# Shuijing725/CrowdNav_Prediction_AttnGraph

Measured on AMD Instinct MI355X. Metric: env-steps/sec (sim+policy fwd) at 20 humans, higher is better.
Workload: dtype f32 (big GEMMs as bf16x3 split-precision MFMA, fp32 accumulate); 1 GPU; BASELINE configs[1]: CrowdSimVarNum-v0, 20 humans, 4096 parallel envs per GPU, HH+HR attention on, policy forward + ORCA sim step + auto-reset per step; envs_per_gpu=4096, humans=20, parallelism=dp1 (envs sharded, no rollout collective), policy_init=orthogonal, torch.manual_seed(425), sampled_actions=True, side_stream_tail=inline, dephase_steps=240

## Files before the change

crowdnav_prediction_attngraph_amd/csrc/orca.h:

```cpp
#pragma once
#include "env_dev.h"
#include "det_math.h"

namespace {

struct LpLine { float px, py, dx, dy; };

__device__ __forceinline__ bool wv_any(bool p) { return __ballot(p) != 0ull; }

__device__ __forceinline__ bool lp1_wave(const LpLine &L, uint64_t valid, int i, float ipx, float ipy, float idx, float idy,
                                         float radius, float optx, float opty, bool dirOpt, int lane, float &rx, float &ry)
{
    const float dotProduct = ipx * idx + ipy * idy;
    const float discriminant = dotProduct * dotProduct + radius * radius - (ipx * ipx + ipy * ipy);
    if (discriminant < 0.0f) return false;
    const float sq = sqrtf(discriminant);
    float tLeft = -dotProduct - sq;
    float tRight = -dotProduct + sq;
    const bool mine = lane < i && ((valid >> lane) & 1ull);
    const float denominator = idx * L.dy - idy * L.dx;
    const float numerator = L.dx * (ipy - L.py) - L.dy * (ipx - L.px);
    const bool parallel = fabsf(denominator) <= RVO_EPS;
    const bool pfail = mine && parallel && numerator < 0.0f;
    const float t = numerator / denominator;
    const float candR = (mine && !parallel && denominator >= 0.0f) ? t : INFINITY;
    const float candL = (mine && !parallel && denominator < 0.0f) ? t : -INFINITY;
    tRight = fminf(tRight, wv_min(candR));
    tLeft = fmaxf(tLeft, wv_max(candL));
    if (wv_any(pfail) || tLeft > tRight) return false;
    float t_opt;
    if (dirOpt) {
        t_opt = (optx * idx + opty * idy > 0.0f) ? tRight : tLeft;
    } else {
        const float tt = idx * (optx - ipx) + idy * (opty - ipy);
        t_opt = tt < tLeft ? tLeft : (tt > tRight ? tRight : tt);
    }
    rx = ipx + t_opt * idx;
    ry = ipy + t_opt * idy;
    return true;
}

__device__ __forceinline__ int lp2_wave(const LpLine &L, uint64_t valid, int n, float radius, float optx, float opty,
                                        bool dirOpt, int lane, float &rx, float &ry)
{
    if (dirOpt) {
        rx = radius * optx; ry = radius * opty;
    } else if (optx * optx + opty * opty > radius * radius) {
        const float inv = 1.0f / sqrtf(optx * optx + opty * opty);
        rx = radius * (optx * inv); ry = radius * (opty * inv);
    } else {
        rx = optx; ry = opty;
    }
    uint64_t todo = valid & (n >= 64 ? ~0ull : ((1ull << n) - 1ull));
    for (;;) {
        const uint64_t vm = __ballot(L.dx * (L.py - ry) - L.dy * (L.px - rx) > 0.0f) & todo;
        if (!vm) return n;
        const int i = __builtin_amdgcn_readfirstlane(__ffsll((unsigned long long)vm) - 1);
        todo &= ~((2ull << i) - 1ull);
        const float ipx = wv_readlane(L.px, i), ipy = wv_readlane(L.py, i);
        const float idx = wv_readlane(L.dx, i), idy = wv_readlane(L.dy, i);
        const float tx = rx, ty = ry;
        if (!lp1_wave(L, valid, i, ipx, ipy, idx, idy, radius, optx, opty, dirOpt, lane, rx, ry)) {
            rx = tx; ry = ty;
            return i;
        }
    }
}

__device__ __forceinline__ void lp3_wave(const LpLine &L, int n, int beginLine, float radius, int lane, float &rx, float &ry)
{
    float distance = 0.0f;
    uint64_t todo = (n >= 64 ? ~0ull : ((1ull << n) - 1ull)) & ~((1ull << beginLine) - 1ull);
    for (;;) {
        const uint64_t vm = __ballot(L.dx * (L.py - ry) - L.dy * (L.px - rx) > distance) & todo;
        if (!vm) return;
        const int i = __builtin_amdgcn_readfirstlane(__ffsll((unsigned long long)vm) - 1);
        todo &= ~((2ull << i) - 1ull);
        const float ipx = wv_readlane(L.px, i), ipy = wv_readlane(L.py, i);
        const float idx = wv_readlane(L.dx, i), idy = wv_readlane(L.dy, i);
        LpLine Pj;
        const float determinant = idx * L.dy - idy * L.dx;
        const bool par = fabsf(determinant) <= RVO_EPS;
        const bool skip = par && (idx * L.dx + idy * L.dy > 0.0f);
        if (par) {
            Pj.px = 0.5f * (ipx + L.px); Pj.py = 0.5f * (ipy + L.py);
        } else {
            const float s = (L.dx * (ipy - L.py) - L.dy * (ipx - L.px)) / determinant;
            Pj.px = ipx + s * idx; Pj.py = ipy + s * idy;
        }
        const float ddx = L.dx - idx, ddy = L.dy - idy;
        const float inv = 1.0f / sqrtf(ddx * ddx + ddy * ddy);
        Pj.dx = ddx * inv; Pj.dy = ddy * inv;
        const uint64_t pvalid = __ballot(lane < i && !skip);
        const float tx = rx, ty = ry;
        if (lp2_wave(Pj, pvalid, i, radius, -idy, idx, true, lane, rx, ry) < i) { rx = tx; ry = ty; }
        distance = idx * (ipy - ry) - idy * (ipx - rx);
    }
}

__device__ __forceinline__ uint32_t hw_ballot(bool p, int lane)
{
    const uint64_t b = __ballot(p);
    return (lane & 32) ? (uint32_t)(b >> 32) : (uint32_t)b;
}
__device__ __forceinline__ float hw_read(float v, int lane, int i)
{
    return __int_as_float(__builtin_amdgcn_ds_bpermute(((lane & 32) + i) << 2, __float_as_int(v)));
}
__device__ __forceinline__ float hw_last(float v, int lane)
{
    const float a = wv_readlane(v, 31), b = wv_readlane(v, 63);
    return (lane & 32) ? b : a;
}
__device__ __forceinline__ uint32_t hw_key(float f)
{
    const uint32_t u = __float_as_uint(f);
    return u ^ ((uint32_t)((int32_t)u >> 31) | 0x80000000u);
}
__device__ __forceinline__ float hw_unkey(uint32_t k) { return __uint_as_float(k ^ ((uint32_t)((int32_t)~k >> 31) | 0x80000000u)); }
template <int CTRL, int ROW_MASK>
__device__ __forceinline__ uint32_t hw_dpp(uint32_t v, uint32_t identity)
{
    return (uint32_t)__builtin_amdgcn_update_dpp((int)identity, (int)v, CTRL, ROW_MASK, 0xf, false);
}
__device__ __forceinline__ uint32_t hw_min(uint32_t v, int lane)
{
    v = min(v, hw_dpp<0x111, 0xf>(v, ~0u));
    v = min(v, hw_dpp<0x112, 0xf>(v, ~0u));
    v = min(v, hw_dpp<0x114, 0xf>(v, ~0u));
    v = min(v, hw_dpp<0x118, 0xf>(v, ~0u));
    v = min(v, hw_dpp<0x142, 0xa>(v, ~0u));
    return __float_as_uint(hw_last(__uint_as_float(v), lane));
}
__device__ __forceinline__ uint32_t hw_max(uint32_t v, int lane)
{
    v = max(v, hw_dpp<0x111, 0xf>(v, 0u));
    v = max(v, hw_dpp<0x112, 0xf>(v, 0u));
    v = max(v, hw_dpp<0x114, 0xf>(v, 0u));
    v = max(v, hw_dpp<0x118, 0xf>(v, 0u));
    v = max(v, hw_dpp<0x142, 0xa>(v, 0u));
    return __float_as_uint(hw_last(__uint_as_float(v), lane));
}

struct LpChord { uint32_t kLeft, kRight, inDisc, pickRight; };

__device__ __forceinline__ LpChord lp_chords(const LpLine &L, float radius, float optx, float opty, int lane)
{
    LpChord c;
    const float dotProduct = L.px * L.dx + L.py * L.dy;
    const float discriminant = dotProduct * dotProduct + radius * radius - (L.px * L.px + L.py * L.py);
    const float sq = sqrtf(discriminant);
    c.kLeft = hw_key(-dotProduct - sq);
    c.kRight = hw_key(-dotProduct + sq);
    c.inDisc = hw_ballot(!(discriminant < 0.0f), lane);
    c.pickRight = hw_ballot(optx * L.dx + opty * L.dy > 0.0f, lane);
    return c;
}

__device__ __forceinline__ bool lp1_pair(const LpLine &L, const LpChord &C, uint32_t valid, int i, float ipx, float ipy, float idx, float idy,
                                         bool act, int lane, float &rx, float &ry)
{
    const int hl = lane & 31;
    bool ok = (C.inDisc >> i) & 1u;
    const uint32_t kLeft = __float_as_uint(hw_read(__uint_as_float(C.kLeft), lane, i));
    const uint32_t kRight = __float_as_uint(hw_read(__uint_as_float(C.kRight), lane, i));
    const bool mine = hl < i && ((valid >> hl) & 1u);
    const float denominator = idx * L.dy - idy * L.dx;
    const float numerator = L.dx * (ipy - L.py) - L.dy * (ipx - L.px);
    const bool parallel = fabsf(denominator) <= RVO_EPS;
    const bool pfail = mine && parallel && numerator < 0.0f;
    const float t = numerator / denominator;
    const uint32_t kt = hw_key(t);
    const uint32_t candR = (mine && !parallel && denominator >= 0.0f) ? kt : 0xff800000u;
    const uint32_t candL = (mine && !parallel && denominator < 0.0f) ? kt : 0x007fffffu;
    const float tRight = hw_unkey(min(kRight, hw_min(candR, lane)));
    const float tLeft = hw_unkey(max(kLeft, hw_max(candL, lane)));
    const uint32_t pf = hw_ballot(pfail, lane);
    ok = ok & (pf == 0u) & !(tLeft > tRight);
    const float t_opt = ((C.pickRight >> i) & 1u) ? tRight : tLeft;
    if (act && ok) {
        rx = ipx + t_opt * idx;
        ry = ipy + t_opt * idy;
    }
    return ok;
}

__device__ __forceinline__ int lp2_pair(const LpLine &L, uint32_t valid, int n, float radius, float optx, float opty, bool act, int lane,
                                        float &rx, float &ry)
{
    if (act) { rx = radius * optx; ry = radius * opty; }
    const LpChord C = lp_chords(L, radius, optx, opty, lane);
    uint32_t todo = valid & ((1u << n) - 1u);
    int res = n;
    bool running = act;
    for (;;) {
        const uint32_t vm = hw_ballot(L.dx * (L.py - ry) - L.dy * (L.px - rx) > 0.0f, lane) & todo;
        const bool go = running && vm != 0u;
        if (__ballot(go) == 0ull) return res;
        running = go;
        const int i = go ? __ffs((int)vm) - 1 : 0;
        if (go) todo &= ~((2u << i) - 1u);
        const float ipx = hw_read(L.px, lane, i), ipy = hw_read(L.py, lane, i);
        const float idx = hw_read(L.dx, lane, i), idy = hw_read(L.dy, lane, i);
        const bool ok = lp1_pair(L, C, valid, i, ipx, ipy, idx, idy, go, lane, rx, ry);
        if (go && !ok) { res = i; running = false; }
    }
}

__device__ __forceinline__ void lp3_pair(const LpLine &L, int n, int beginLine, float radius, bool act, int lane, float &rx, float &ry)
{
    const int hl = lane & 31;
    float distance = 0.0f;
    uint32_t todo = (n >= 32 ? ~0u : ((1u << n) - 1u)) & ~((1u << beginLine) - 1u);
    bool running = act;
    for (;;) {
        const uint32_t vm = hw_ballot(L.dx * (L.py - ry) - L.dy * (L.px - rx) > distance, lane) & todo;
        const bool go = running && vm != 0u;
        if (__ballot(go) == 0ull) return;
        running = go;
        const int i = go ? __ffs((int)vm) - 1 : 0;
        if (go) todo &= ~((2u << i) - 1u);
        const float ipx = hw_read(L.px, lane, i), ipy = hw_read(L.py, lane, i);
        const float idx = hw_read(L.dx, lane, i), idy = hw_read(L.dy, lane, i);
        LpLine Pj;
        const float determinant = idx * L.dy - idy * L.dx;
        const bool par = fabsf(determinant) <= RVO_EPS;
        const bool skip = par && (idx * L.dx + idy * L.dy > 0.0f);
        if (par) {
            Pj.px = 0.5f * (ipx + L.px); Pj.py = 0.5f * (ipy + L.py);
        } else {
            const float s = (L.dx * (ipy - L.py) - L.dy * (ipx - L.px)) / determinant;
            Pj.px = ipx + s * idx; Pj.py = ipy + s * idy;
        }
        const float ddx = L.dx - idx, ddy = L.dy - idy;
        const float inv = 1.0f / sqrtf(ddx * ddx + ddy * ddy);
        Pj.dx = ddx * inv; Pj.dy = ddy * inv;
        const uint32_t pvalid = hw_ballot(hl < i && !skip, lane);
        const float tx = rx, ty = ry;
        const int f = lp2_pair(Pj, pvalid, i, radius, -idy, idx, go, lane, rx, ry);
        if (go && f < i) { rx = tx; ry = ty; }
        if (go) distance = idx * (ipy - ry) - idy * (ipx - rx);
    }
}

__global__ __launch_bounds__(256) void orca_lp3_kernel(EnvDev s)
{
    const CnStampScope stamp_scope(s.stamp);
    const int lane = threadIdx.x & 63, hl = lane & 31, half = lane >> 5;
    const int total = *s.lp3_cnt;
    const int pairs = (total + 1) >> 1;
    const int H = s.H;
    for (int p = __builtin_amdgcn_readfirstlane(blockIdx.x * 4 + (threadIdx.x >> 6)); p < pairs; p += gridDim.x * 4) {
        const bool act = 2 * p + half < total;
        const int k = act ? 2 * p + half : 2 * p;
        const Lp3Hdr hd = s.lp3_hdr[k];
        float4 raw = s.lp3_lines[(size_t)k * 32 + hl];
        raw.x = held(raw.x); raw.y = held(raw.y); raw.z = held(raw.z); raw.w = held(raw.w);
        const float4 ln = hl < hd.nn ? raw : make_float4(0.0f, 0.0f, 1.0f, 0.0f);
        LpLine L;
        L.px = ln.x; L.py = ln.y; L.dx = ln.z; L.dy = ln.w;
        float rx = hd.rx, ry = hd.ry;
        lp3_pair(L, hd.nn, hd.line_fail, hd.radius, act, lane, rx, ry);
        if (act && hl == 0) {
            const int e = hd.agent / H, i = hd.agent - e * H;
            s.hact[(size_t)e * 2 * H + i] = rx;
            s.hact[(size_t)e * 2 * H + H + i] = ry;
        }
    }
}

__device__ __forceinline__ void orca_wave(int lane, int nl, bool cand, float opx, float opy, float ovx, float ovy, float orad,
                                          float spx, float spy, float svx, float svy, float srad, float maxspeed, float prefx,
                                          float prefy, float nd, int max_nb, float th, float dt, float &outx, float &outy)
{
    const float ddx0 = spx - opx, ddy0 = spy - opy;
    const float dq = ddx0 * ddx0 + ddy0 * ddy0;
    const bool inrange = cand && dq < nd * nd;
    const float key = inrange ? dq : INFINITY;
    int rank = 0;
    for (int m = 0; m < nl; ++m) {
        const float km = wv_readlane(key, m);
        rank += (km < key || (km == key && m < lane)) ? 1 : 0;
    }
    if (lane >= nl) rank = lane;
    int nn = __popcll(__ballot(inrange));
    if (nn > max_nb) nn = max_nb;
    const float rpx = opx - spx, rpy = opy - spy;
    const float rvx = svx - ovx, rvy = svy - ovy;
    const float distSq = rpx * rpx + rpy * rpy;
    const float cr = srad + orad;
    const float crSq = cr * cr;
    float ldx, ldy, ux, uy;
    if (distSq > crSq) {
        const float invTH = 1.0f / th;
        const float wx = rvx - invTH * rpx, wy = rvy - invTH * rpy;
        const float wLenSq = wx * wx + wy * wy;
        const float dot1 = wx * rpx + wy * rpy;
        if (dot1 < 0.0f && dot1 * dot1 > crSq * wLenSq) {
            const float wLen = sqrtf(wLenSq);
            const float inv = 1.0f / wLen;
            const float uwx = wx * inv, uwy = wy * inv;
            ldx = uwy; ldy = -uwx;
            const float s = cr * invTH - wLen;
            ux = s * uwx; uy = s * uwy;
        } else {
            const float leg = sqrtf(distSq - crSq);
            const float invD = 1.0f / distSq;
            if (rpx * wy - rpy * wx > 0.0f) {
                ldx = (rpx * leg - rpy * cr) * invD;
                ldy = (rpx * cr + rpy * leg) * invD;
            } else {
                ldx = -((rpx * leg + rpy * cr) * invD);
                ldy = -((-rpx * cr + rpy * leg) * invD);
            }
            const float dot2 = rvx * ldx + rvy * ldy;
            ux = dot2 * ldx - rvx; uy = dot2 * ldy - rvy;
        }
    } else {
        const float invDT = 1.0f / dt;
        const float wx = rvx - invDT * rpx, wy = rvy - invDT * rpy;
        const float wLen = sqrtf(wx * wx + wy * wy);
        const float inv = 1.0f / wLen;
        const float uwx = wx * inv, uwy = wy * inv;
        ldx = uwy; ldy = -uwx;
        const float s = cr * invDT - wLen;
        ux = s * uwx; uy = s * uwy;
    }
    const float lpx = svx + 0.5f * ux, lpy = svy + 0.5f * uy;
    LpLine L;
    L.px = __int_as_float(__builtin_amdgcn_ds_permute(rank << 2, __float_as_int(lpx)));
    L.py = __int_as_float(__builtin_amdgcn_ds_permute(rank << 2, __float_as_int(lpy)));
    L.dx = __int_as_float(__builtin_amdgcn_ds_permute(rank << 2, __float_as_int(ldx)));
    L.dy = __int_as_float(__builtin_amdgcn_ds_permute(rank << 2, __float_as_int(ldy)));
    const uint64_t valid = nn >= 64 ? ~0ull : ((1ull << nn) - 1ull);
    float rx, ry;
    const int lineFail = lp2_wave(L, valid, nn, maxspeed, prefx, prefy, false, lane, rx, ry);
    if (lineFail < nn) lp3_wave(L, nn, lineFail, maxspeed, lane, rx, ry);
    outx = rx; outy = ry;
}

__device__ __forceinline__ void orca_agent(const EnvDev &s, int agent, int lane)
{
    const int H = s.H;
    const int e = agent / H, i = agent - e * H;
    const int n = crowd_size(s, e);
    if (i >= n) return;
    const double *hum = s.hum + (size_t)e * 8 * H;
    const bool isH = lane < n;
    const int lj = isH ? lane : 0;
    const double px = hum[F_PX * H + lj], py = hum[F_PY * H + lj], vx = hum[F_VX * H + lj], vy = hum[F_VY * H + lj];
    const double rad = hum[F_RAD * H + lj];
    const double spx = __shfl(px, i, 64), spy = __shfl(py, i, 64), svx = __shfl(vx, i, 64), svy = __shfl(vy, i, 64);
    const double sgx = hum[F_GX * H + i], sgy = hum[F_GY * H + i], srad = hum[F_RAD * H + i], svpref = hum[F_VPREF * H + i];
    const double safety = s.cfg.orca_safety_space;
    const size_t ei = (size_t)e * H + i;
    float nd, self_r, self_ms, seen_r;
    const bool rv = s.cfg.robot_visible != 0;
    const int n_agents = n + (rv ? 1 : 0);
    const bool isR = rv && lane == n;
    const double *rob = s.rob + (size_t)e * 8;
    const double qx = isR ? rob[R_PX] : px, qy = isR ? rob[R_PY] : py, qvx = isR ? rob[R_VX] : vx, qvy = isR ? rob[R_VY] : vy;
    const bool coincident = s.cfg.human_fov < 2.0 ? !in_fov(s.cfg, s.cfg.human_fov, spx, spy, svx, svy, 0.0, qx, qy) : (qx == spx) && (qy == spy);
    if (!s.sim_valid[ei] || (s.sim_n && s.sim_n[ei] != n_agents)) {
        nd = (float)s.shared_nd[e];
        self_r = (float)(srad + 0.01 + safety);
        self_ms = (float)svpref;
        seen_r = (float)((coincident ? s.cfg.human_radius : rad) + 0.01 + safety);
        if (s.sim_seen && isH) s.sim_seen[ei * H + lane] = seen_r;
        if (lane == 0) {
            s.sim_nd[ei] = nd; s.sim_self_radius[ei] = self_r; s.sim_self_maxspeed[ei] = self_ms; s.sim_valid[ei] = 1;
            if (s.sim_n) s.sim_n[ei] = (uint8_t)n_agents;
        }
    } else {
        nd = s.sim_nd[ei]; self_r = s.sim_self_radius[ei]; self_ms = s.sim_self_maxspeed[ei];
        seen_r = s.sim_seen ? s.sim_seen[ei * H + lj] : (float)(rad + 0.01 + safety);
    }
    if (isR) seen_r = (float)(s.cfg.robot_radius + 0.01 + safety);
    const bool cand = (isH && lane != i) || isR;
    const float opx = coincident ? 7.0f : (float)qx, opy = coincident ? 7.0f : (float)qy;
    const float ovx = coincident ? 0.0f : (float)qvx, ovy = coincident ? 0.0f : (float)qvy;
    double gvx = sgx - spx, gvy = sgy - spy;
    const double speed = sqrt(gvx * gvx + gvy * gvy);
    if (speed > 1.0) { gvx = gvx / speed; gvy = gvy / speed; }
    float ox, oy;
    orca_wave(lane, n_agents, cand, opx, opy, ovx, ovy, seen_r, (float)spx, (float)spy, (float)svx, (float)svy, self_r, self_ms,
              (float)gvx, (float)gvy, nd, n_agents - 1, (float)s.cfg.orca_time_horizon, (float)s.cfg.time_step, ox, oy);
    if (lane == 0) {
        s.hact[(size_t)e * 2 * H + i] = ox;
        s.hact[(size_t)e * 2 * H + H + i] = oy;
    }
}

__global__ __launch_bounds__(256) void orca_kernel(EnvDev s)
{
    const CnStampScope stamp_scope(s.stamp);
    const int lane = threadIdx.x & 63;
    const int total = s.E * s.H;
    for (int agent = __builtin_amdgcn_readfirstlane(blockIdx.x * 4 + (threadIdx.x >> 6)); agent < total; agent += gridDim.x * 4)
        orca_agent(s, agent, lane);
}

#include "orca_sortnet.inc"
#include "row_plan.h"

template <int W> struct LaneVec;
template <> struct LaneVec<8> { typedef float f __attribute__((ext_vector_type(8))); };
template <> struct LaneVec<32> { typedef float f __attribute__((ext_vector_type(32))); };

template <int NB, int VW>
__global__ __launch_bounds__(64) void orca_lane_kernel(EnvDev s, const float *plan_det, int32_t *plan, int plan_groups, unsigned long long *plan_stamp)
{
    const CnStampScope stamp_scope((plan && (int)blockIdx.x < plan_groups) ? plan_stamp : s.stamp);
    constexpr int RAW = (int)sizeof(rowplan::Lds) > NB * 64 * 16 ? (int)sizeof(rowplan::Lds) : NB * 64 * 16;
    __shared__ __attribute__((aligned(16))) char s_raw[RAW];
    if (plan && (int)blockIdx.x < plan_groups) {
        __builtin_amdgcn_s_setprio(3);
        rowplan::build((int)blockIdx.x, plan_groups, s.E, s.H, rp_workgroups(s.E, s.H), plan_det, plan, *reinterpret_cast<rowplan::Lds *>(s_raw), nullptr, s.plan_arrive);
        return;
    }
    const int blk = (int)blockIdx.x - (plan ? plan_groups : 0);
    typedef typename LaneVec<VW>::f vec;
    const int agent = blk * 64 + threadIdx.x;
    const int H = s.H;
    const bool live_lane = agent < s.E * H;
    const int e = live_lane ? agent / H : (blk * 64) / H, i = live_lane ? agent - e * H : 0;
    const int n = crowd_size(s, e);
    const bool active = live_lane && i < n;
    const cn_env_config &c = s.cfg;
    constexpr int NENV = NB == 8 ? 65 : (NB == 20 ? 10 : 5);
    __shared__ double s_px[128], s_py[128], s_vx[128], s_vy[128], s_rad[128], s_rob[NENV][4];
    const double *hum = s.hum + (size_t)e * 8 * H;
    const size_t ei = (size_t)e * H + i;
    double sgx, sgy, svpref, shared_nd_in;
    int sim_valid_in, sim_n_in = 0;
    float sim_nd_in, sim_r_in, sim_ms_in;
    {
        const int a0 = blk * 64;
        const int e0 = a0 / H, e1 = (min(a0 + 63, s.E * H - 1)) / H;
        const int nrows = (e1 - e0 + 1) * H;
        double st[2][5];
#pragma unroll
        for (int it = 0; it < 2; ++it) {
            const int r = threadIdx.x + 64 * it;
            if (r < nrows) {
                const int ee = e0 + r / H, j = r - (r / H) * H;
                const double *hm = s.hum + (size_t)ee * 8 * H;
                st[it][0] = hm[F_PX * H + j]; st[it][1] = hm[F_PY * H + j]; st[it][2] = hm[F_VX * H + j]; st[it][3] = hm[F_VY * H + j];
                st[it][4] = hm[F_RAD * H + j];
            }
        }
        sgx = hum[F_GX * H + i]; sgy = hum[F_GY * H + i]; svpref = hum[F_VPREF * H + i];
        sim_valid_in = s.sim_valid[ei];
        if (s.sim_n) sim_n_in = s.sim_n[ei];
        sim_nd_in = s.sim_nd[ei]; sim_r_in = s.sim_self_radius[ei]; sim_ms_in = s.sim_self_maxspeed[ei];
        shared_nd_in = s.shared_nd[e];
#pragma unroll
        for (int it = 0; it < 2; ++it) {
            const int r = threadIdx.x + 64 * it;
            if (r < nrows) { s_px[r] = st[it][0]; s_py[r] = st[it][1]; s_vx[r] = st[it][2]; s_vy[r] = st[it][3]; s_rad[r] = st[it][4]; }
        }
        if (c.robot_visible)
            for (int q = threadIdx.x; q <= e1 - e0; q += 64) {
                const double *rb = s.rob + (size_t)(e0 + q) * 8;
                s_rob[q][0] = rb[R_PX]; s_rob[q][1] = rb[R_PY]; s_rob[q][2] = rb[R_VX]; s_rob[q][3] = rb[R_VY];
            }
        __syncthreads();
    }
    const int eq = e - (blk * 64) / H, eb = eq * H;
    const double spx = s_px[eb + i], spy = s_py[eb + i], svx = s_vx[eb + i], svy = s_vy[eb + i], srad = s_rad[eb + i];
    const double safety = c.orca_safety_space;
    const bool rv = c.robot_visible != 0;
    const int n_agents = n + (rv ? 1 : 0);
    float nd = 0.0f, self_r = 0.0f, self_ms = 0.0f;
    if (active) {
        const bool rebuild = !sim_valid_in || (s.sim_n && sim_n_in != n_agents);
        if (rebuild) {
            nd = (float)shared_nd_in;
            self_r = (float)(srad + 0.01 + safety);
            self_ms = (float)svpref;
            if (s.sim_seen)
                for (int j = 0; j < n; ++j) s.sim_seen[ei * H + j] = (float)(s_rad[eb + j] + 0.01 + safety);
            s.sim_nd[ei] = nd; s.sim_self_radius[ei] = self_r; s.sim_self_maxspeed[ei] = self_ms; s.sim_valid[ei] = 1;
            if (s.sim_n) s.sim_n[ei] = (uint8_t)n_agents;
        } else {
            nd = sim_nd_in; self_r = sim_r_in; self_ms = sim_ms_in;
        }
    }
    const float fpx = (float)spx, fpy = (float)spy, fvx = (float)svx, fvy = (float)svy;
    vec key, idx;
    int nn = 0;
#pragma unroll 1
    for (int j = 0; j < NB; ++j) {
        const bool isR = rv && j == n;
        const bool cand = active && ((j < n && j != i) || isR);
        const int lj = j < n ? j : 0;
        const double qx = isR ? s_rob[eq][0] : s_px[eb + lj], qy = isR ? s_rob[eq][1] : s_py[eb + lj];
        const bool coincident = (qx == spx) && (qy == spy);
        const float opx = coincident ? 7.0f : (float)qx, opy = coincident ? 7.0f : (float)qy;
        const float ddx0 = fpx - opx, ddy0 = fpy - opy;
        const float dq = ddx0 * ddx0 + ddy0 * ddy0;
        const bool inrange = cand && dq < nd * nd;
        key[j] = inrange ? dq : INFINITY;
        idx[j] = (float)j;
        nn += inrange ? 1 : 0;
    }
#define ORCA_CE(a, b)                                                                                  \
    {                                                                                                  \
        const float ka0 = key[a], kb0 = key[b], ia0 = idx[a], ib0 = idx[b];                             \
        const bool sw = kb0 < ka0 || (kb0 == ka0 && ib0 < ia0);                                         \
        key[a] = sw ? kb0 : ka0; key[b] = sw ? ka0 : kb0; idx[a] = sw ? ib0 : ia0; idx[b] = sw ? ia0 : ib0; \
    }
    if constexpr (NB == 8) { ORCA_SORTNET_8(ORCA_CE) }
    else if constexpr (NB == 20) { ORCA_SORTNET_20(ORCA_CE) }
    else { static_assert(NB == 32, "sorting networks exist for 8, 20 and 32 slots"); ORCA_SORTNET_32(ORCA_CE) }
#undef ORCA_CE
    int nmax = nn;
    for (int off = 32; off >= 1; off >>= 1) nmax = max(nmax, __shfl_xor(nmax, off, 64));
    nmax = __builtin_amdgcn_readfirstlane(nmax);
    const float invTH = 1.0f / (float)c.orca_time_horizon, invDT = 1.0f / (float)c.time_step;
    float4 *const s_line = reinterpret_cast<float4 *>(s_raw);
    const int tid = threadIdx.x;
#pragma unroll 1
    for (int k = 0; k < nmax; ++k) {
        float o_px = 0.0f, o_py = 0.0f, o_dx = 1.0f, o_dy = 0.0f;
        const int j = (int)idx[k];
        if (k < nn) {
            const bool isR = j == n;
            const int lj = isR ? 0 : j;
            const double qx = isR ? s_rob[eq][0] : s_px[eb + lj], qy = isR ? s_rob[eq][1] : s_py[eb + lj];
            const double qvx = isR ? s_rob[eq][2] : s_vx[eb + lj], qvy = isR ? s_rob[eq][3] : s_vy[eb + lj];
            float orad;
            if (isR) orad = (float)(c.robot_radius + 0.01 + safety);
            else if (s.sim_seen) orad = s.sim_seen[ei * H + lj];
            else orad = (float)(s_rad[eb + lj] + 0.01 + safety);
            const bool coincident = (qx == spx) && (qy == spy);
            const float opx = coincident ? 7.0f : (float)qx, opy = coincident ? 7.0f : (float)qy;
            const float ovx = coincident ? 0.0f : (float)qvx, ovy = coincident ? 0.0f : (float)qvy;
            const float rpx = opx - fpx, rpy = opy - fpy;
            const float rvx = fvx - ovx, rvy = fvy - ovy;
            const float distSq = rpx * rpx + rpy * rpy;
            const float cr = self_r + orad;
            const float crSq = cr * cr;
            const bool collide = !(distSq > crSq);
            const float invT = collide ? invDT : invTH;
            const float wx = rvx - invT * rpx, wy = rvy - invT * rpy;
            const float wLenSq = wx * wx + wy * wy;
            const float dot1 = wx * rpx + wy * rpy;
            const bool circle = collide || (dot1 < 0.0f && dot1 * dot1 > crSq * wLenSq);
            const float sq = sqrtf(circle ? wLenSq : distSq - crSq);
            const float inv = 1.0f / (circle ? sq : distSq);
            const float uwx = wx * inv, uwy = wy * inv;
            const float sc = cr * invT - sq;
            const bool left = rpx * wy - rpy * wx > 0.0f;
            const float lgx = left ? (rpx * sq - rpy * cr) * inv : -((rpx * sq + rpy * cr) * inv);
            const float lgy = left ? (rpx * cr + rpy * sq) * inv : -((-rpx * cr + rpy * sq) * inv);
            const float dot2 = rvx * lgx + rvy * lgy;
            const float ldx = circle ? uwy : lgx, ldy = circle ? -uwx : lgy;
            const float ux = circle ? sc * uwx : dot2 * lgx - rvx, uy = circle ? sc * uwy : dot2 * lgy - rvy;
            o_px = fvx + 0.5f * ux; o_py = fvy + 0.5f * uy; o_dx = ldx; o_dy = ldy;
        }
        s_line[k * 64 + tid] = make_float4(o_px, o_py, o_dx, o_dy);
    }
    double gvx = sgx - spx, gvy = sgy - spy;
    const double speed = sqrt(gvx * gvx + gvy * gvy);
    if (speed > 1.0) { gvx = gvx / speed; gvy = gvy / speed; }
    const float optx = (float)gvx, opty = (float)gvy, radius = self_ms;
    float rx, ry;
    if (optx * optx + opty * opty > radius * radius) {
        const float inv = 1.0f / sqrtf(optx * optx + opty * opty);
        rx = radius * (optx * inv); ry = radius * (opty * inv);
    } else {
        rx = optx; ry = opty;
    }
    unsigned *const s_tl = reinterpret_cast<unsigned *>(s_line + (NB - 1) * 64), *const s_tr = s_tl + 64;
    int *const s_pf = reinterpret_cast<int *>(s_tr + 64), *const s_vl = s_pf + 64;
    auto okey = [](float f) { const unsigned u = __float_as_uint(f); return u ^ ((u >> 31) ? 0xffffffffu : 0x80000000u); };
    auto okey_inv = [](unsigned o) { return __uint_as_float(o ^ ((o >> 31) ? 0x80000000u : 0xffffffffu)); };
    bool failed = false;
    int line_fail = 0;
#pragma unroll 1
    for (int li = 0; li < nmax; ++li) {
        const float4 Li = s_line[li * 64 + tid];
        const float ipx = Li.x, ipy = Li.y, idx_ = Li.z, idy = Li.w;
        const bool viol = li < nn && !failed && idx_ * (ipy - ry) - idy * (ipx - rx) > 0.0f;
        const unsigned long long vm = __ballot(viol);
        if (vm == 0ull) continue;
        const float dotProduct = ipx * idx_ + ipy * idy;
        const float discriminant = dotProduct * dotProduct + radius * radius - (ipx * ipx + ipy * ipy);
        bool ok = !(discriminant < 0.0f);
        const float sq = sqrtf(discriminant);
        float tLeft = -dotProduct - sq, tRight = -dotProduct + sq;
        bool pfail = false;
        const int npairs = __popcll(vm) * li;
        if (npairs > 0) {
            if (viol) {
                const int rank = __builtin_amdgcn_mbcnt_hi((unsigned)(vm >> 32), __builtin_amdgcn_mbcnt_lo((unsigned)vm, 0u));
                s_vl[rank] = tid; s_tl[tid] = okey(tLeft); s_tr[tid] = okey(tRight); s_pf[tid] = 0;
            }
            __syncthreads();
            const unsigned inv20 = ((1u << 20) + (unsigned)li - 1u) / (unsigned)li;
#pragma unroll 1
            for (int p0 = 0; p0 < npairs; p0 += 64) {
                const int p = p0 + tid;
                const bool on = p < npairs;
                const int r = on ? (int)(((unsigned)p * inv20) >> 20) : 0;
                const int lj = on ? p - r * li : 0;
                const int a = s_vl[r];
                const float4 A = s_line[li * 64 + a], B = s_line[lj * 64 + a];
                const float denominator = A.z * B.w - A.w * B.z;
                const float numerator = B.z * (A.y - B.y) - B.w * (A.x - B.x);
                const bool parallel = fabsf(denominator) <= RVO_EPS;
                const float t = numerator / denominator;
                if (on) {
                    if (parallel) { if (numerator < 0.0f) s_pf[a] = 1; }
                    else if (denominator >= 0.0f) atomicMin(&s_tr[a], okey(t));
                    else atomicMax(&s_tl[a], okey(t));
                }
            }
            __syncthreads();
            if (viol) { tLeft = okey_inv(s_tl[tid]); tRight = okey_inv(s_tr[tid]); pfail = s_pf[tid] != 0; }
            __syncthreads();
        }
        ok = ok && !pfail && !(tLeft > tRight);
        if (viol) {
            if (ok) {
                const float tt = idx_ * (optx - ipx) + idy * (opty - ipy);
                const float t_opt = tt < tLeft ? tLeft : (tt > tRight ? tRight : tt);
                rx = ipx + t_opt * idx_;
                ry = ipy + t_opt * idy;
            } else {
                failed = true;
                line_fail = li;
            }
        }
    }
    int slot = -1;
    if (active && failed) {
        slot = atomicAdd(s.lp3_cnt, 1);
        Lp3Hdr hd;
        hd.agent = agent; hd.nn = nn; hd.line_fail = line_fail; hd.rx = rx; hd.ry = ry; hd.radius = radius;
        s.lp3_hdr[slot] = hd;
    } else if (active) {
        s.hact[(size_t)e * 2 * H + i] = rx;
        s.hact[(size_t)e * 2 * H + H + i] = ry;
    }
    if (__ballot(slot >= 0) != 0ull) {
#pragma unroll 1
        for (int k = 0; k < nmax; ++k) {
            const float4 ln = s_line[k * 64 + tid];
            if (slot >= 0 && k < nn) s.lp3_lines[(size_t)slot * 32 + k] = ln;
        }
    }
}

__global__ __launch_bounds__(256) void orca_truth_kernel(EnvDev s, int k)
{
    const int lane = threadIdx.x & 63;
    const int agent = __builtin_amdgcn_readfirstlane(blockIdx.x * 4 + (threadIdx.x >> 6));
    if (agent >= s.E * s.H) return;
    const int H = s.H;
    const int e = agent / H, i = agent - e * H;
    const int n = crowd_size(s, e);
    if (i >= n) return;
    const double *hum = s.hum + (size_t)e * 8 * H;
    double *trk = s.tr + ((size_t)e * (s.R + 1) + k) * 4 * H;
    const double *src = k == 1 ? hum : trk - 4 * H;
    const bool isH = lane < n;
    const int lj = isH ? lane : 0;
    const double px = src[0 * H + lj], py = src[1 * H + lj], vx = src[2 * H + lj], vy = src[3 * H + lj];
    const double rad = hum[F_RAD * H + lj];
    const double spx = __shfl(px, i, 64), spy = __shfl(py, i, 64), svx = __shfl(vx, i, 64), svy = __shfl(vy, i, 64);
    const double sgx = hum[F_GX * H + i], sgy = hum[F_GY * H + i];
    const size_t ei = (size_t)e * H + i;
    float nd, self_r, self_ms, seen_r;
    if (!s.sim_valid[ei] || (s.sim_n && s.sim_n[ei] != n)) {
        const double safety = s.cfg.orca_safety_space;
        nd = (float)s.shared_nd[e];
        self_r = (float)(hum[F_RAD * H + i] + 0.01 + safety);
        self_ms = (float)hum[F_VPREF * H + i];
        seen_r = (float)(rad + 0.01 + safety);
        if (s.sim_seen && isH) s.sim_seen[ei * H + lane] = seen_r;
        if (lane == 0) {
            s.sim_nd[ei] = nd; s.sim_self_radius[ei] = self_r; s.sim_self_maxspeed[ei] = self_ms; s.sim_valid[ei] = 1;
            if (s.sim_n) s.sim_n[ei] = (uint8_t)n;
        }
    } else {
        nd = s.sim_nd[ei]; self_r = s.sim_self_radius[ei]; self_ms = s.sim_self_maxspeed[ei];
        seen_r = s.sim_seen ? s.sim_seen[ei * H + lj] : (float)(rad + 0.01 + s.cfg.orca_safety_space);
    }
    const bool cand = isH && lane != i;
    double gvx = sgx - spx, gvy = sgy - spy;
    const double speed = sqrt(gvx * gvx + gvy * gvy);
    if (speed > 1.0) { gvx = gvx / speed; gvy = gvy / speed; }
    float ox, oy;
    orca_wave(lane, n, cand, (float)px, (float)py, (float)vx, (float)vy, seen_r, (float)spx, (float)spy, (float)svx, (float)svy, self_r, self_ms,
              (float)gvx, (float)gvy, nd, n - 1, (float)s.cfg.orca_time_horizon, (float)s.cfg.time_step, ox, oy);
    if (lane == 0) {
        trk[0 * H + i] = spx + (double)ox * s.cfg.time_step;
        trk[1 * H + i] = spy + (double)oy * s.cfg.time_step;
        trk[2 * H + i] = (double)ox;
        trk[3 * H + i] = (double)oy;
    }
}

__global__ __launch_bounds__(64) void sf_truth_kernel(EnvDev s)
{
    const int e = blockIdx.x, lane = threadIdx.x;
    const int H = s.H, n = crowd_size(s, e);
    const cn_env_config &c = s.cfg;
    const double *hum = s.hum + (size_t)e * 8 * H;
    const bool isH = lane < n;
    const int lj = isH ? lane : 0;
    double px = hum[F_PX * H + lj], py = hum[F_PY * H + lj], vx = hum[F_VX * H + lj], vy = hum[F_VY * H + lj];
    const double rad = hum[F_RAD * H + lj], gx = hum[F_GX * H + lj], gy = hum[F_GY * H + lj], vpref = hum[F_VPREF * H + lj];
    for (int k = 1; k <= s.R; ++k) {
        const double dxg = gx - px, dyg = gy - py;
        const double dist_to_goal = sqrt(dxg * dxg + dyg * dyg);
        const double desired_vx = (dxg / dist_to_goal) * vpref, desired_vy = (dyg / dist_to_goal) * vpref;
        const double curr_dvx = c.sf_KI * (desired_vx - vx), curr_dvy = c.sf_KI * (desired_vy - vy);
        double ivx = 0.0, ivy = 0.0;
        for (int j = 0; j < n; ++j) {
            const double ox = __shfl(px, j, 64), oy = __shfl(py, j, 64), orad = __shfl(rad, j, 64);
            const double dx = px - ox, dy = py - oy;
            const double d = sqrt(dx * dx + dy * dy);
            const double f = c.sf_A * det_exp((rad + orad - d) / c.sf_B);
            if (j != lane) { ivx += f * (dx / d); ivy += f * (dy / d); }
        }
        const double nvx = vx + (curr_dvx + ivx) * c.time_step, nvy = vy + (curr_dvy + ivy) * c.time_step;
        const double act_norm = sqrt(nvx * nvx + nvy * nvy);
        double ax = nvx, ay = nvy;
        if (act_norm > vpref) { ax = nvx / act_norm * vpref; ay = nvy / act_norm * vpref; }
        px = px + ax * c.time_step; py = py + ay * c.time_step; vx = ax; vy = ay;
        if (isH) {
            double *trk = s.tr + ((size_t)e * (s.R + 1) + k) * 4 * H;
            trk[0 * H + lane] = px; trk[1 * H + lane] = py; trk[2 * H + lane] = vx; trk[3 * H + lane] = vy;
        }
    }
}

__global__ __launch_bounds__(256) void orca_solve_kernel(int B, int n_other, const float *self, const float *others, float nd,
                                                         int max_nb, float th, float dt, float *out)
{
    const int lane = threadIdx.x & 63;
    const int b = __builtin_amdgcn_readfirstlane(blockIdx.x * 4 + (threadIdx.x >> 6));
    if (b >= B) return;
    const float *sp = self + (size_t)b * 8;
    const bool cand = lane < n_other;
    const float *o = others + ((size_t)b * n_other + (cand ? lane : 0)) * 5;
    float ox, oy;
    orca_wave(lane, n_other, cand, o[0], o[1], o[2], o[3], o[4], sp[0], sp[1], sp[2], sp[3], sp[4], sp[5], sp[6], sp[7], nd,
              max_nb, th, dt, ox, oy);
    if (lane == 0) { out[2 * b] = ox; out[2 * b + 1] = oy; }
}

}
```

Before: 16.91 million env-steps/s.

## Repack ORCA lane-kernel neighbor data into float4 LDS records and integer sort slots

Reorganizes the ORCA per-lane kernel's shared-memory staging so the robot occupies an extra row per env, with precomputed float4 position/velocity records and combined radii, replacing separate double arrays and a special robot branch. The neighbor sort now uses packed unsigned key/index pairs compared as a 64-bit value, and coincidence flags are cached in a bitmask instead of being recomputed. The per-line reciprocal divisor is taken from a constant table via readlane instead of an integer divide. This cuts LDS traffic, double conversions and divide latency, at the cost of more register-held sort state and more complex indexing.

```diff
diff --git a/crowdnav_prediction_attngraph_amd/csrc/orca.h b/crowdnav_prediction_attngraph_amd/csrc/orca.h
--- a/crowdnav_prediction_attngraph_amd/csrc/orca.h
+++ b/crowdnav_prediction_attngraph_amd/csrc/orca.h
@@ -403,9 +403,45 @@
 #include "orca_sortnet.inc"
 #include "row_plan.h"
 
-template <int W> struct LaneVec;
-template <> struct LaneVec<8> { typedef float f __attribute__((ext_vector_type(8))); };
-template <> struct LaneVec<32> { typedef float f __attribute__((ext_vector_type(32))); };
+template <int NB> struct SortSlots {
+    static constexpr int LO = NB < 16 ? NB : 16, HI = NB > 16 ? 16 : 0;
+    typedef unsigned lo_w __attribute__((ext_vector_type(2 * LO)));
+    typedef unsigned hi_w __attribute__((ext_vector_type(HI ? 2 * HI : 2)));
+    lo_w lo;
+    hi_w hi;
+    template <int A> __device__ __forceinline__ unsigned idx() const { if constexpr (A < LO) return lo[2 * A]; else return hi[2 * (A - LO)]; }
+    template <int A> __device__ __forceinline__ unsigned key() const { if constexpr (A < LO) return lo[2 * A + 1]; else return hi[2 * (A - LO) + 1]; }
+    template <int A> __device__ __forceinline__ void set(unsigned k, unsigned i)
+    {
+        if constexpr (A < LO) { lo[2 * A] = i; lo[2 * A + 1] = k; } else { hi[2 * (A - LO)] = i; hi[2 * (A - LO) + 1] = k; }
+    }
+    template <int A> __device__ __forceinline__ void init_indices()
+    {
+        set<A>(0u, (unsigned)A);
+        if constexpr (A + 1 < NB) init_indices<A + 1>();
+    }
+    template <int A, int B> __device__ __forceinline__ void exchange()
+    {
+        const unsigned ka = key<A>(), ia = idx<A>(), kb = key<B>(), ib = idx<B>();
+        const bool sw = ((unsigned long long)kb << 32 | ib) < ((unsigned long long)ka << 32 | ia);
+        set<A>(sw ? kb : ka, sw ? ib : ia); set<B>(sw ? ka : kb, sw ? ia : ib);
+    }
+    template <class V, int A = 0> __device__ __forceinline__ void order(V &v) const
+    {
+        v[A] = idx<A>();
+        if constexpr (A + 1 < NB) order<V, A + 1>(v);
+    }
+};
+
+constexpr unsigned orca_inv20(unsigned li) { return li ? ((1u << 20) + li - 1u) / li : 0u; }
+struct OrcaInv20 { unsigned v[32]; };
+constexpr OrcaInv20 orca_inv20_table()
+{
+    OrcaInv20 t{};
+    for (unsigned li = 0; li < 32; ++li) t.v[li] = orca_inv20(li);
+    return t;
+}
+__constant__ const OrcaInv20 k_orca_inv20 = orca_inv20_table();
 
 template <int NB, int VW>
 __global__ __launch_bounds__(64) void orca_lane_kernel(EnvDev s, const float *plan_det, int32_t *plan, int plan_groups, unsigned long long *plan_stamp)
@@ -419,7 +455,6 @@
         return;
     }
     const int blk = (int)blockIdx.x - (plan ? plan_groups : 0);
-    typedef typename LaneVec<VW>::f vec;
     const int agent = blk * 64 + threadIdx.x;
     const int H = s.H;
     const bool live_lane = agent < s.E * H;
@@ -427,26 +462,37 @@
     const int n = crowd_size(s, e);
     const bool active = live_lane && i < n;
     const cn_env_config &c = s.cfg;
-    constexpr int NENV = NB == 8 ? 65 : (NB == 20 ? 10 : 5);
-    __shared__ double s_px[128], s_py[128], s_vx[128], s_vy[128], s_rad[128], s_rob[NENV][4];
+    __shared__ double s_px[128], s_py[128];
+    __shared__ float4 s_rec[128];
+    __shared__ float s_crad[128];
+    const double safety = c.orca_safety_space;
+    const bool rv = c.robot_visible != 0;
+    const int HS = H + (rv ? 1 : 0);
     const double *hum = s.hum + (size_t)e * 8 * H;
     const size_t ei = (size_t)e * H + i;
     double sgx, sgy, svpref, shared_nd_in;
     int sim_valid_in, sim_n_in = 0;
     float sim_nd_in, sim_r_in, sim_ms_in;
+    unsigned inv20_lane;
     {
         const int a0 = blk * 64;
         const int e0 = a0 / H, e1 = (min(a0 + 63, s.E * H - 1)) / H;
-        const int nrows = (e1 - e0 + 1) * H;
+        const int nrows = (e1 - e0 + 1) * HS;
         double st[2][5];
 #pragma unroll
         for (int it = 0; it < 2; ++it) {
             const int r = threadIdx.x + 64 * it;
             if (r < nrows) {
-                const int ee = e0 + r / H, j = r - (r / H) * H;
-                const double *hm = s.hum + (size_t)ee * 8 * H;
-                st[it][0] = hm[F_PX * H + j]; st[it][1] = hm[F_PY * H + j]; st[it][2] = hm[F_VX * H + j]; st[it][3] = hm[F_VY * H + j];
-                st[it][4] = hm[F_RAD * H + j];
+                const int ee = e0 + r / HS, j = r - (r / HS) * HS;
+                if (j < H) {
+                    const double *hm = s.hum + (size_t)ee * 8 * H;
+                    st[it][0] = hm[F_PX * H + j]; st[it][1] = hm[F_PY * H + j]; st[it][2] = hm[F_VX * H + j]; st[it][3] = hm[F_VY * H + j];
+                    st[it][4] = hm[F_RAD * H + j];
+                } else {
+                    const double *rb = s.rob + (size_t)ee * 8;
+                    st[it][0] = rb[R_PX]; st[it][1] = rb[R_PY]; st[it][2] = rb[R_VX]; st[it][3] = rb[R_VY];
+                    st[it][4] = c.robot_radius;
+                }
             }
         }
         sgx = hum[F_GX * H + i]; sgy = hum[F_GY * H + i]; svpref = hum[F_VPREF * H + i];
@@ -454,88 +500,90 @@
         if (s.sim_n) sim_n_in = s.sim_n[ei];
         sim_nd_in = s.sim_nd[ei]; sim_r_in = s.sim_self_radius[ei]; sim_ms_in = s.sim_self_maxspeed[ei];
         shared_nd_in = s.shared_nd[e];
+        inv20_lane = k_orca_inv20.v[threadIdx.x & 31];
 #pragma unroll
         for (int it = 0; it < 2; ++it) {
             const int r = threadIdx.x + 64 * it;
-            if (r < nrows) { s_px[r] = st[it][0]; s_py[r] = st[it][1]; s_vx[r] = st[it][2]; s_vy[r] = st[it][3]; s_rad[r] = st[it][4]; }
-        }
-        if (c.robot_visible)
-            for (int q = threadIdx.x; q <= e1 - e0; q += 64) {
-                const double *rb = s.rob + (size_t)(e0 + q) * 8;
-                s_rob[q][0] = rb[R_PX]; s_rob[q][1] = rb[R_PY]; s_rob[q][2] = rb[R_VX]; s_rob[q][3] = rb[R_VY];
+            if (r < nrows) {
+                s_px[r] = st[it][0]; s_py[r] = st[it][1];
+                s_rec[r] = make_float4((float)st[it][0], (float)st[it][1], (float)st[it][2], (float)st[it][3]);
+                s_crad[r] = (float)(st[it][4] + 0.01 + safety);
             }
+        }
         __syncthreads();
     }
-    const int eq = e - (blk * 64) / H, eb = eq * H;
-    const double spx = s_px[eb + i], spy = s_py[eb + i], svx = s_vx[eb + i], svy = s_vy[eb + i], srad = s_rad[eb + i];
-    const double safety = c.orca_safety_space;
-    const bool rv = c.robot_visible != 0;
+    const int eb = (e - (blk * 64) / H) * HS;
+    const double spx = s_px[eb + i], spy = s_py[eb + i];
+    const float4 own = s_rec[eb + i];
     const int n_agents = n + (rv ? 1 : 0);
     float nd = 0.0f, self_r = 0.0f, self_ms = 0.0f;
     if (active) {
         const bool rebuild = !sim_valid_in || (s.sim_n && sim_n_in != n_agents);
         if (rebuild) {
             nd = (float)shared_nd_in;
-            self_r = (float)(srad + 0.01 + safety);
+            self_r = s_crad[eb + i];
             self_ms = (float)svpref;
             if (s.sim_seen)
-                for (int j = 0; j < n; ++j) s.sim_seen[ei * H + j] = (float)(s_rad[eb + j] + 0.01 + safety);
+                for (int j = 0; j < n; ++j) s.sim_seen[ei * H + j] = s_crad[eb + j];
             s.sim_nd[ei] = nd; s.sim_self_radius[ei] = self_r; s.sim_self_maxspeed[ei] = self_ms; s.sim_valid[ei] = 1;
             if (s.sim_n) s.sim_n[ei] = (uint8_t)n_agents;
         } else {
             nd = sim_nd_in; self_r = sim_r_in; self_ms = sim_ms_in;
         }
     }
-    const float fpx = (float)spx, fpy = (float)spy, fvx = (float)svx, fvy = (float)svy;
-    vec key, idx;
+    const float fpx = own.x, fpy = own.y, fvx = own.z, fvy = own.w;
+    SortSlots<NB> slots;
+    slots.template init_indices<0>();
+    unsigned cmask = 0u;
     int nn = 0;
-#pragma unroll 1
-    for (int j = 0; j < NB; ++j) {
-        const bool isR = rv && j == n;
-        const bool cand = active && ((j < n && j != i) || isR);
-        const int lj = j < n ? j : 0;
-        const double qx = isR ? s_rob[eq][0] : s_px[eb + lj], qy = isR ? s_rob[eq][1] : s_py[eb + lj];
-        const bool coincident = (qx == spx) && (qy == spy);
-        const float opx = coincident ? 7.0f : (float)qx, opy = coincident ? 7.0f : (float)qy;
+    const int rob_row = rv ? H : 0;
+    const int n_cand = active ? n_agents : 0;
+    auto key_of = [&](int j) {
+        const bool cand = j < n_cand && j != i;
+        const int row = eb + (j < n ? j : rob_row);
+        const double qx = s_px[row], qy = s_py[row];
+        const float2 qf = *reinterpret_cast<const float2 *>(&s_rec[row]);
+        const bool coincident = (qx == spx) & (qy == spy);
+        cmask |= coincident ? 1u << j : 0u;
+        const float opx = coincident ? 7.0f : qf.x, opy = coincident ? 7.0f : qf.y;
         const float ddx0 = fpx - opx, ddy0 = fpy - opy;
         const float dq = ddx0 * ddx0 + ddy0 * ddy0;
         const bool inrange = cand && dq < nd * nd;
-        key[j] = inrange ? dq : INFINITY;
-        idx[j] = (float)j;
         nn += inrange ? 1 : 0;
-    }
-#define ORCA_CE(a, b)                                                                                  \
-    {                                                                                                  \
-        const float ka0 = key[a], kb0 = key[b], ia0 = idx[a], ib0 = idx[b];                             \
-        const bool sw = kb0 < ka0 || (kb0 == ka0 && ib0 < ia0);                                         \
-        key[a] = sw ? kb0 : ka0; key[b] = sw ? ka0 : kb0; idx[a] = sw ? ib0 : ia0; idx[b] = sw ? ia0 : ib0; \
-    }
+        return __float_as_uint(inrange ? dq : INFINITY);
+    };
+#pragma unroll 1
+    for (int j = 0; j < SortSlots<NB>::LO; ++j) slots.lo[2 * j + 1] = key_of(j);
+    if constexpr (SortSlots<NB>::HI != 0) {
+#pragma unroll 1
+        for (int j = SortSlots<NB>::LO; j < NB; ++j) slots.hi[2 * (j - SortSlots<NB>::LO) + 1] = key_of(j);
+    }
+#define ORCA_CE(a, b) slots.template exchange<a, b>();
     if constexpr (NB == 8) { ORCA_SORTNET_8(ORCA_CE) }
     else if constexpr (NB == 20) { ORCA_SORTNET_20(ORCA_CE) }
     else { static_assert(NB == 32, "sorting networks exist for 8, 20 and 32 slots"); ORCA_SORTNET_32(ORCA_CE) }
 #undef ORCA_CE
+    typedef unsigned order_t __attribute__((ext_vector_type(VW)));
+    order_t order;
+    slots.template order<order_t>(order);
     int nmax = nn;
     for (int off = 32; off >= 1; off >>= 1) nmax = max(nmax, __shfl_xor(nmax, off, 64));
     nmax = __builtin_amdgcn_readfirstlane(nmax);
-    const float invTH = 1.0f / (float)c.orca_time_horizon, invDT = 1.0f / (float)c.time_step;
+    const float invTH = held_uniform(1.0f / (float)c.orca_time_horizon), invDT = held_uniform(1.0f / (float)c.time_step);
     float4 *const s_line = reinterpret_cast<float4 *>(s_raw);
     const int tid = threadIdx.x;
 #pragma unroll 1
     for (int k = 0; k < nmax; ++k) {
         float o_px = 0.0f, o_py = 0.0f, o_dx = 1.0f, o_dy = 0.0f;
-        const int j = (int)idx[k];
+        const int j = (int)order[k];
         if (k < nn) {
-            const bool isR = j == n;
-            const int lj = isR ? 0 : j;
-            const double qx = isR ? s_rob[eq][0] : s_px[eb + lj], qy = isR ? s_rob[eq][1] : s_py[eb + lj];
-            const double qvx = isR ? s_rob[eq][2] : s_vx[eb + lj], qvy = isR ? s_rob[eq][3] : s_vy[eb + lj];
-            float orad;
-            if (isR) orad = (float)(c.robot_radius + 0.01 + safety);
-            else if (s.sim_seen) orad = s.sim_seen[ei * H + lj];
-            else orad = (float)(s_rad[eb + lj] + 0.01 + safety);
-            const bool coincident = (qx == spx) && (qy == spy);
-            const float opx = coincident ? 7.0f : (float)qx, opy = coincident ? 7.0f : (float)qy;
-            const float ovx = coincident ? 0.0f : (float)qvx, ovy = coincident ? 0.0f : (float)qvy;
+            const int row = eb + (j == n ? H : j);
+            const float4 q = s_rec[row];
+            float orad = s_crad[row];
+            if (s.sim_seen && j != n) orad = s.sim_seen[ei * H + j];
+            const bool coincident = (cmask >> j) & 1u;
+            const float opx = coincident ? 7.0f : q.x, opy = coincident ? 7.0f : q.y;
+            const float ovx = coincident ? 0.0f : q.z, ovy = coincident ? 0.0f : q.w;
             const float rpx = opx - fpx, rpy = opy - fpy;
             const float rvx = fvx - ovx, rvy = fvy - ovy;
             const float distSq = rpx * rpx + rpy * rpy;
@@ -580,6 +628,7 @@
     int line_fail = 0;
 #pragma unroll 1
     for (int li = 0; li < nmax; ++li) {
+        const unsigned inv20 = (unsigned)__builtin_amdgcn_readlane((int)inv20_lane, li);
         const float4 Li = s_line[li * 64 + tid];
         const float ipx = Li.x, ipy = Li.y, idx_ = Li.z, idy = Li.w;
         const bool viol = li < nn && !failed && idx_ * (ipy - ry) - idy * (ipx - rx) > 0.0f;
@@ -598,7 +647,6 @@
                 s_vl[rank] = tid; s_tl[tid] = okey(tLeft); s_tr[tid] = okey(tRight); s_pf[tid] = 0;
             }
             __syncthreads();
-            const unsigned inv20 = ((1u << 20) + (unsigned)li - 1u) / (unsigned)li;
 #pragma unroll 1
             for (int p0 = 0; p0 < npairs; p0 += 64) {
                 const int p = p0 + tid;
```

Result: no change. 17.04 million env-steps/s (median of 6 runs) (+0.8%).
